# chaudatascience/diverse_channel_vit

Hardware: AMD Instinct MI355X
Metric: train images/sec, DiChaViT-S 8ch 224^2 bs=64/GPU (higher is better)
Workload: dtype bf16; 1 GPU; DiChaViT-small 8ch 224x224 P16 161 classes, train step (fwd + CE + ortho/proxy regularisers + bwd + fused AdamW), bs 64/GPU, N=1569 tokens; global_batch=64, seq_len=1569, parallelism=dp1, input=resident in HBM, launch=eager, wgrad_stream=False, wgrad_group=True

## Files before the change

### diverse_channel_vit_amd/csrc/gemm.hip

```cpp
#include <algorithm>
#include <atomic>
#include <type_traits>
#include "dcv_common.hpp"
#include "../../include/dcv.h"

namespace {

constexpr int BK = 64;

struct GemmNtArgs {
    const bf16_t* A;
    int lda;
    const bf16_t* W;
    int ldw;
    int M, N, K;
    const float* bias;
    void* out;
    int ldo;
    void* out2;
    int ldo2;
    const void* aux;
    int ldaux;
    const float* aux2;
    int T, n;
// ... 554 lines not shown
                const int c = 2 * hc + q;
                f32x4 va, vb;
#pragma unroll
                for (int r = 0; r < 4; ++r) {
                    float fa, fbv;
                    xchg_rows8(acc[i][2 * c][r], acc[i][2 * c + 1][r], fa, fbv);
                    va[r] = fa;
                    vb[r] = fbv;
                }
                const float bq[4] = {b4[q].x, b4[q].y, b4[q].z, b4[q].w};
                const float pa[4] = {xa[q].x, xa[q].y, xa[q].z, xa[q].w}, pb[4] = {xb[q].x, xb[q].y, xb[q].z, xb[q].w};
#pragma unroll
                for (int r = 0; r < 4; ++r) {
                    va[r] = fmaf(sa, va[r] + bq[r], pa[r]);
                    vb[r] = fmaf(sb, vb[r] + bq[r], pb[r]);
                }
                acc[i][2 * c] = va;
                acc[i][2 * c + 1] = vb;
                if (ma < a.M) *reinterpret_cast<f32x4*>((float*)a.out + (size_t)ma * a.ldo + ncol0 + 32 * c) = va;
                if (mb < a.M) *reinterpret_cast<f32x4*>((float*)a.out + (size_t)mb * a.ldo + ncol0 + 32 * c) = vb;
            }
        }
        float mu[2], m2[2];
#pragma unroll
        for (int h = 0; h < 2; ++h) {
            float s = 0.f;
#pragma unroll
            for (int c = 0; c < 6; ++c)
#pragma unroll
                for (int r = 0; r < 4; ++r) s += acc[i][2 * c + h][r];
            const float m = s * (1.f / 24.f);
            float q = 0.f;
#pragma unroll
            for (int c = 0; c < 6; ++c)
#pragma unroll
                for (int r = 0; r < 4; ++r) {
                    const float d = acc[i][2 * c + h][r] - m;
                    q = fmaf(d, d, q);
                }
            mu[h] = m;
            m2[h] = q;
        }
        float half_n = 12.f;
#pragma unroll
        for (int off = 8; off <= 32; off <<= 1) {
#pragma unroll
            for (int h = 0; h < 2; ++h) {
                const float om = __shfl_xor(mu[h], off, 64), oq = __shfl_xor(m2[h], off, 64);
                const float d = om - mu[h];
                m2[h] = m2[h] + oq + d * d * half_n;
                mu[h] = 0.5f * (mu[h] + om);
            }
            half_n *= 2.f;
        }
        if (hi == 0 && kg == 0) {
            const int rl = 16 * RB * wm + 16 * i + rr;
            *reinterpret_cast<float2*>(stat + ((size_t)(wn * 256 + rl) * 2)) = make_float2(mu[0], m2[0]);
            *reinterpret_cast<float2*>(stat + ((size_t)(wn * 256 + rl + 8) * 2)) = make_float2(mu[1], m2[1]);
        }
    }
    {
        const int t = 64 * (2 * wm + wn) + ln;
        if (t < 192) {
            const float4 v = *reinterpret_cast<const float4*>((t < 96 ? a.ln_g : a.ln_b) + 4 * (t < 96 ? t : t - 96));
            *reinterpret_cast<float4*>(stat + 1024 + 4 * t) = v;
        }
    }
    asm volatile("s_waitcnt lgkmcnt(0)" ::: "memory");
    __builtin_amdgcn_s_barrier();
    const int ln2 = lane_id_here();
    const int kg2 = ln2 >> 4, rr2 = ln2 & 7, hi2 = (ln2 >> 3) & 1;
    const int ncol2 = 192 * wn + 16 * hi2 + 4 * kg2;
#pragma unroll
    for (int i = 0; i < RB; ++i) {
        const int ma = m0 + 16 * RB * wm + 16 * i + rr2, mb = ma + 8;
        const int rl = 16 * RB * wm + 16 * i + rr2;
        float mean[2], rstd[2];
#pragma unroll
        for (int h = 0; h < 2; ++h) {
            const float2 p0 = *reinterpret_cast<const float2*>(stat + ((size_t)(rl + 8 * h) * 2));
            const float2 p1 = *reinterpret_cast<const float2*>(stat + ((size_t)(256 + rl + 8 * h) * 2));
            const float d = p1.x - p0.x;
            mean[h] = 0.5f * (p0.x + p1.x);
            rstd[h] = rsqrtf((p0.y + p1.y + d * d * 96.f) * (1.f / 384.f) + a.ln_eps);
        }
        if (wn == 0 && hi2 == 0 && kg2 == 0) {
            if (ma < a.M) { a.ln_mean[ma] = mean[0]; a.ln_rstd[ma] = rstd[0]; }
            if (mb < a.M) { a.ln_mean[mb] = mean[1]; a.ln_rstd[mb] = rstd[1]; }
        }
#pragma unroll
        for (int hc = 0; hc < 3; ++hc) {
            float4 g4[2], be4[2];
#pragma unroll
            for (int q = 0; q < 2; ++q) {
                g4[q] = *reinterpret_cast<const float4*>(stat + 1024 + ncol2 + 32 * (2 * hc + q));
                be4[q] = *reinterpret_cast<const float4*>(stat + 1024 + 384 + ncol2 + 32 * (2 * hc + q));
            }
            uint2 pa[2], pb[2];
#pragma unroll
            for (int q = 0; q < 2; ++q) {
                const int c = 2 * hc + q;
                const float g[4] = {g4[q].x, g4[q].y, g4[q].z, g4[q].w}, be[4] = {be4[q].x, be4[q].y, be4[q].z, be4[q].w};
                float ua[4], ub[4];
#pragma unroll
                for (int r = 0; r < 4; ++r) {
                    ua[r] = fmaf((acc[i][2 * c][r] - mean[0]) * rstd[0], g[r], be[r]);
                    ub[r] = fmaf((acc[i][2 * c + 1][r] - mean[1]) * rstd[1], g[r], be[r]);
                }
                pa[q] = pack4_bf16(ua[0], ua[1], ua[2], ua[3]);
                pb[q] = pack4_bf16(ub[0], ub[1], ub[2], ub[3]);
            }
            const u32x2_t ax = __builtin_amdgcn_permlane16_swap(pa[0].x, pa[1].x, false, false);
            const u32x2_t ay = __builtin_amdgcn_permlane16_swap(pa[0].y, pa[1].y, false, false);
            const u32x2_t bx = __builtin_amdgcn_permlane16_swap(pb[0].x, pb[1].x, false, false);
            const u32x2_t by = __builtin_amdgcn_permlane16_swap(pb[0].y, pb[1].y, false, false);
            const int kgp = kg2 & 1;
            const int ucol = 192 * wn + 32 * (2 * hc + kgp) + 16 * hi2 + 4 * (kg2 - kgp);
            if (ma < a.M) *reinterpret_cast<uint4*>((bf16_t*)a.out2 + (size_t)ma * a.ldo2 + ucol) = make_uint4(ax[0], ay[0], ax[1], ay[1]);
            if (mb < a.M) *reinterpret_cast<uint4*>((bf16_t*)a.out2 + (size_t)mb * a.ldo2 + ucol) = make_uint4(bx[0], by[0], bx[1], by[1]);
        }
    }
}

constexpr int N3_BM = 256, N3_BN = 384, N3_BK = 64;
constexpr int N3_A_BYTES = N3_BM * N3_BK * 2, N3_W_BYTES = N3_BN * N3_BK * 2, N3_STAGE_BYTES = N3_A_BYTES + N3_W_BYTES;
constexpr int N3_SMEM = 2 * N3_STAGE_BYTES;

template <int EPI>
__global__ __launch_bounds__(512) void gemm_nt384_kernel(GemmNtArgs a) {
    __shared__ __attribute__((aligned(16))) char smem[N3_SMEM];
    constexpr bool HAS_BIAS = (EPI != DCV_EPI_PLAIN_BF16) && (EPI != DCV_EPI_GELU_BWD_BF16);
    static_assert(EPI != DCV_EPI_PATCH, "the tokeniser epilogue stays on the 256 x 128 kernel");
    constexpr bool LN = (EPI == DCV_EPI_RESID_LN);
    constexpr int S1 = LN ? 0 : 3 * nt_stores_per_wave<LN ? DCV_EPI_BIAS_RESID_F32 : EPI>() / 4;
    const int tid = threadIdx.x, lane = tid & 63;
    const int wave = __builtin_amdgcn_readfirstlane(tid >> 6);
    const int wm = wave >> 1, wn = wave & 1;
    const bool late = (wave >> 2) != 0;
    const int tiles_n = a.N / N3_BN;
    const int total = a.tiles_m * tiles_n;
    const int G = gridDim.x;
    const int pos = ((G & 7) == 0) ? (blockIdx.x & 7) * (G >> 3) + (blockIdx.x >> 3) : blockIdx.x;

    const unsigned smem_base = __builtin_amdgcn_readfirstlane(lds_addr(smem));
    const unsigned dmaA = 32 * wave * 128, dmaW = N3_A_BYTES + 48 * wave * 128;
    const int nk = a.K / N3_BK;
    __builtin_assume(nk >= 1);
    const int r16 = lane & 15, kg = lane >> 4;
    const int rowA = (wm * 64 + r16) * 128, rowW = N3_A_BYTES + (wn * 192 + r16) * 128;
    int fA0, fA1, fW0, fW1;
    {
        const int co0 = (kg ^ swz64n(r16)) << 4;
        fA0 = rowA + co0; fA1 = rowA + (co0 ^ 64); fW0 = rowW + co0; fW1 = rowW + (co0 ^ 64);
        asm volatile("" : "+v"(fA0), "+v"(fA1), "+v"(fW0), "+v"(fW1));
    }

    unsigned voffA[2], voffW[2];
    auto set_voff = [&]() {
        const int ln = lane_id_here();
#pragma unroll
        for (int q = 0; q < 2; ++q) {
            const int rowa = 32 * wave + 8 * q + (ln >> 3), roww = 48 * wave + 8 * q + (ln >> 3);
            voffA[q] = (unsigned)(((size_t)rowa * a.lda + (((ln & 7) ^ swz64n(rowa)) * 8)) * 2);
            voffW[q] = (unsigned)(((size_t)roww * a.ldw + (((ln & 7) ^ swz64n(roww)) * 8)) * 2);
        }
    };
    set_voff();
    auto issue = [&](int m0_, int n0_, int h_, int kt, unsigned stage_base) {
        const int m0 = __builtin_amdgcn_readfirstlane(m0_), n0 = __builtin_amdgcn_readfirstlane(n0_);
        const int h = __builtin_amdgcn_readfirstlane(h_);
        const bf16_t* ab = a.A + (size_t)m0 * a.lda + kt * N3_BK;
        const bf16_t* wb = a.W + (size_t)n0 * a.ldw + kt * N3_BK;
        const bool has_rows = 32 * wave < h;
        if (has_rows && m0 + h <= a.M) {
#pragma unroll
            for (int q = 0; q < 4; ++q) glds16s(ab + (size_t)(q >> 1) * 16 * a.lda, voffA[q & 1], stage_base + dmaA + q * 1024);
        } else if (has_rows) {
            const int ln = lane_id_here();
#pragma unroll
            for (int q = 0; q < 4; ++q) {
                const int row = 32 * wave + 8 * q + (ln >> 3);
                const int rc = min(m0 + row, a.M - 1) - m0;
                glds16s(ab, (unsigned)(((size_t)rc * a.lda + (((ln & 7) ^ swz64n(row)) * 8)) * 2), stage_base + dmaA + q * 1024);
            }
        }
#pragma unroll
        for (int q = 0; q < 6; ++q) glds16s(wb + (size_t)(q >> 1) * 16 * a.ldw, voffW[q & 1], stage_base + dmaW + q * 1024);
    };

    auto tile_at = [&](int L_, int& m0_, int& n0_, int& h_) {
        const int tm = L_ / tiles_n, s192 = tm - a.n256;
        m0_ = s192 < 0 ? tm * N3_BM : a.n256 * N3_BM + s192 * 192;
        h_ = s192 < 0 ? N3_BM : 192;
        n0_ = (L_ - tm * tiles_n) * N3_BN;
    };
    int L = pos < total ? pos : -1;
    int Lnext = (L >= 0 && L + G < total) ? L + G : -1;
    if (L < 0) return;
    int m0, n0, h;
    tile_at(L, m0, n0, h);
    int g = 0;
    issue(m0, n0, h, 0, smem_base);
    int stores_behind = 0;

    auto tile = [&](auto rbc) __attribute__((always_inline)) -> bool {
        constexpr int RB = decltype(rbc)::value;
        constexpr int H = 64 * RB;
        f32x4 acc[RB][12];
#pragma unroll
        for (int i = 0; i < RB; ++i)
#pragma unroll
            for (int j = 0; j < 12; ++j)
#pragma unroll
                for (int r = 0; r < 4; ++r) acc[i][j][r] = 0.f;

#pragma clang loop unroll(disable)
        for (int kt = 0; kt < nk; ++kt, ++g) {
            if (kt == 0 && stores_behind == 4) asm volatile("s_waitcnt vmcnt(%0)" ::"n"(4 * S1) : "memory");
            else if (kt == 0 && stores_behind == 3) asm volatile("s_waitcnt vmcnt(%0)" ::"n"(3 * S1) : "memory");
            else asm volatile("s_waitcnt vmcnt(0)" ::: "memory");
            __builtin_amdgcn_s_barrier();
            const char* st = smem + (g & 1) * N3_STAGE_BYTES;
            const char* const stA = st - (4 - RB) * wm * 16 * 128;
            const char* const pA0 = stA + fA0;
            const char* const pA1 = stA + fA1;
            const char* const pW0 = st + fW0;
            const char* const pW1 = st + fW1;
            auto rdW = [&](int s2) { return as_bf16x8(lds_read128(s2 >= 12 ? pW1 : pW0, (s2 % 12) * 16 * 128)); };
            bf16x8 af[RB], wq[3];
#pragma unroll
            for (int i = 0; i < RB; ++i) af[i] = as_bf16x8(lds_read128(pA0, i * 16 * 128));
            wq[0] = rdW(0);
            wq[1] = rdW(1);
            __builtin_amdgcn_sched_barrier(0);
            if (kt + 1 < nk && (DCV_N3_EARLY_AT < 0 || late)) issue(m0, n0, H, kt + 1, smem_base + ((g + 1) & 1) * N3_STAGE_BYTES);
            __builtin_amdgcn_sched_barrier(0);
#pragma unroll
            for (int s2 = 0; s2 < 24; ++s2) {
                if (s2 + 2 < 24) wq[(s2 + 2) % 3] = rdW(s2 + 2);
#pragma unroll
                for (int i = 0; i < RB; ++i) {
                    acc[i][s2 % 12] = mfma16(wq[s2 % 3], af[i], acc[i][s2 % 12]);
                    if (s2 == 11) af[i] = as_bf16x8(lds_read128(pA1, i * 16 * 128));
                }
                __builtin_amdgcn_sched_barrier(0);
                if (DCV_N3_EARLY_AT >= 0 && s2 == DCV_N3_EARLY_AT) {
                    if (kt + 1 < nk && !late) issue(m0, n0, H, kt + 1, smem_base + ((g + 1) & 1) * N3_STAGE_BYTES);
                    __builtin_amdgcn_sched_barrier(0);
                }
            }
        }

        const int Ln = Lnext;
        const bool has_next = Ln >= 0;
        int m0n = 0, n0n = 0, hn = N3_BM;
        if (has_next) tile_at(Ln, m0n, n0n, hn);
        Lnext = (has_next && Ln + G < total) ? Ln + G : -1;
        const bool full = (m0 + H <= a.M);
        const int m_w = m0 + wm * 16 * RB, n_w = n0 + wn * 192;
        const int ln = lane_id_here();
        const int r16e = ln & 15, kge = ln >> 4;
        if constexpr (LN) {
            nt384_resid_ln_epilogue<RB>(a, acc, m0, wm, wn, ln, smem + ((g + 1) & 1) * N3_STAGE_BYTES, [&]() {
                if (has_next) issue(m0n, n0n, hn, 0, smem_base + (g & 1) * N3_STAGE_BYTES);
            });
        } else {
            auto block = [&](auto j0c, auto&& between) {
                constexpr int J0 = decltype(j0c)::value;
                float bz[8];
                if constexpr (HAS_BIAS) nt_load_bias<EPI, 4>(a, n_w + 16 * J0, r16e, kge, bz);
                nt_epilogue_block<EPI, 1, 4, 12, J0>(a, acc, m_w, n_w + 16 * J0, r16e, kge, bz, between);
            };
            block(std::integral_constant<int, 0>{}, [&]() {
                if (has_next) issue(m0n, n0n, hn, 0, smem_base + (g & 1) * N3_STAGE_BYTES);
            });
            block(std::integral_constant<int, 4>{}, []() {});
            block(std::integral_constant<int, 8>{}, []() {});
        }
        if (!has_next) return false;
        stores_behind = (full && !LN) ? RB : 0;
        m0 = m0n;
        n0 = n0n;
        h = hn;
        L = Ln;
        set_voff();
        return true;
    };
    for (;;) {
        if (h == N3_BM) {
            if (!tile(std::integral_constant<int, 4>{})) break;
        } else {
            if (!tile(std::integral_constant<int, 3>{})) break;
        }
    }
}

#ifndef DCV_NT_WS
#define DCV_NT_WS 1
#endif
#if DCV_NT_WS
constexpr int WS_BM = 32, WS_BN = 384, WS_K = 384, WS_WAVES = 12;
constexpr int WS_A_BYTES = WS_BM * WS_K * 2;
constexpr int WS_AUX_BYTES = WS_BM * WS_BN * 2;
template <int EPI>
struct WsCfg {
    static constexpr bool AUX = (EPI == DCV_EPI_GELU_BWD_BF16);
    static constexpr int STAGE = WS_A_BYTES + (AUX ? WS_AUX_BYTES : 0);
    static constexpr int NS = AUX ? 3 : 6;
    static constexpr int ND = AUX ? 4 : 2;
    static constexpr int S = 2 * (EPI == DCV_EPI_BIAS_GELU_BF16 ? 2 : 1);
    static constexpr int SMEM = NS * STAGE;
};

__device__ __forceinline__ void ws_wait_vm(int n) {
    switch (n) {
#define WS_W(k) \
    case k: asm volatile("s_waitcnt vmcnt(" #k ")" ::: "memory"); break;
        WS_W(0) WS_W(1) WS_W(2) WS_W(3) WS_W(4) WS_W(5) WS_W(6) WS_W(7) WS_W(8) WS_W(9) WS_W(10) WS_W(11) WS_W(12)
        WS_W(13) WS_W(14) WS_W(15) WS_W(16) WS_W(17) WS_W(18) WS_W(19) WS_W(20) WS_W(21) WS_W(22) WS_W(23) WS_W(24)
#undef WS_W
        default: asm volatile("s_waitcnt vmcnt(0)" ::: "memory"); break;
    }
}

template <int EPI>
__global__ __launch_bounds__(64 * WS_WAVES) void gemm_nt_ws_kernel(GemmNtArgs a) {
    using C = WsCfg<EPI>;
    __shared__ __attribute__((aligned(16))) char smem[C::SMEM];
    constexpr bool HAS_BIAS = (EPI == DCV_EPI_BIAS_BF16) || (EPI == DCV_EPI_BIAS_GELU_BF16);
    static_assert(EPI == DCV_EPI_BIAS_BF16 || EPI == DCV_EPI_BIAS_GELU_BF16 || EPI == DCV_EPI_PLAIN_BF16 || EPI == DCV_EPI_GELU_BWD_BF16,
                  "bf16-output epilogues only");
    const int tid = threadIdx.x, lane = tid & 63;
    const int wave = __builtin_amdgcn_readfirstlane(tid >> 6);
    const int r16 = lane & 15, kg = lane >> 4;
    const int slices = a.N / WS_BN;
    const int G = gridDim.x;
    const int groups = G / slices;
    const int q = xcd_remap(blockIdx.x, G);
    const int slice = q % slices, grp = q / slices;
    const int panels = (a.M + WS_BM - 1) / WS_BM;
    const int npl = grp < panels ? (panels - grp + groups - 1) / groups : 0;
    if (npl == 0) return;
    const int n0 = slice * WS_BN, nw = n0 + 32 * wave;
    const int ncol = nw + 16 * (kg & 1) + 8 * (kg >> 1);

    const unsigned smem_base = __builtin_amdgcn_readfirstlane(lds_addr(smem));
    int arow[2];
    unsigned acol[2], adst[2];
#pragma unroll
    for (int u = 0; u < 2; ++u) {
        const int p = 2 * wave + u, kc = p >> 2, row = 8 * (p & 3) + (lane >> 3);
        arow[u] = row;
        acol[u] = (unsigned)(64 * kc + (((lane & 7) ^ swz64n(row)) * 8)) * 2;
        adst[u] = kc * 4096 + (p & 3) * 1024;
    }
    auto issue = [&](int t) {
        const int m0 = __builtin_amdgcn_readfirstlane((grp + t * groups) * WS_BM);
        const unsigned slot = smem_base + (t % C::NS) * C::STAGE;
        const bf16_t* ab = a.A + (size_t)m0 * a.lda;
#pragma unroll
        for (int u = 0; u < 2; ++u) {
            const int rc = min(m0 + arow[u], a.M - 1) - m0;
            glds16s(ab, (unsigned)rc * a.lda * 2 + acol[u], slot + adst[u]);
        }
        if constexpr (C::AUX) {
            const bf16_t* xb = (const bf16_t*)a.aux + (size_t)m0 * a.ldaux;
#pragma unroll
            for (int i = 0; i < 2; ++i) {
                const int rc = min(m0 + 16 * i + r16, a.M - 1) - m0;
                glds16s(xb, (unsigned)(rc * a.ldaux + ncol) * 2, slot + WS_A_BYTES + (2 * wave + i) * 1024);
            }
        }
    };

    bf16x8 wf[2][12];
#pragma unroll
    for (int j = 0; j < 2; ++j) {
        const bf16_t* wr = a.W + (size_t)(nw + 16 * j + r16) * a.ldw + 8 * kg;
#pragma unroll
        for (int s = 0; s < 12; ++s) wf[j][s] = as_bf16x8(*reinterpret_cast<const uint4*>(wr + 32 * s));
    }
    float bz[8];
    if constexpr (HAS_BIAS) load8_f32(a.bias + ncol, bz);
#pragma unroll
    for (int t = 0; t < C::NS - 1; ++t)
        if (t < npl) issue(t);
#pragma unroll
    for (int j = 0; j < 2; ++j)
#pragma unroll
        for (int s = 0; s < 12; ++s) asm volatile("" : "+v"(wf[j][s]));
    if constexpr (HAS_BIAS) {
#pragma unroll
        for (int e = 0; e < 8; ++e) asm volatile("" : "+v"(bz[e]));
    }

    int fo0 = r16 * 128 + ((kg ^ swz64n(r16)) << 4);
    asm volatile("" : "+v"(fo0));
    const int fo1 = fo0 ^ 64;
    bool prev_full = false;
    for (int t = 0; t < npl; ++t) {
        const int ahead = min(C::NS - 2, npl - 1 - t);
        ws_wait_vm(C::ND * ahead + (prev_full ? C::S : 0));
        __builtin_amdgcn_s_barrier();
        if (t + C::NS - 1 < npl) issue(t + C::NS - 1);
        const int m0 = (grp + t * groups) * WS_BM;
        const char* st = smem + (t % C::NS) * C::STAGE;
        const char* const p0 = st + fo0;
        const char* const p1 = st + fo1;

        f32x4 acc[2][2];
#pragma unroll
        for (int i = 0; i < 2; ++i)
#pragma unroll
            for (int j = 0; j < 2; ++j)
#pragma unroll
                for (int r = 0; r < 4; ++r) acc[i][j][r] = 0.f;
        auto rdA = [&](int s, int i) { return as_bf16x8(lds_read128((s & 1) ? p1 : p0, (s >> 1) * 4096 + i * 2048)); };
        bf16x8 af[2][2];
        af[0][0] = rdA(0, 0);
        af[0][1] = rdA(0, 1);
#pragma unroll
        for (int s = 0; s < 12; ++s) {
            if (s + 1 < 12) {
                af[(s + 1) & 1][0] = rdA(s + 1, 0);
                af[(s + 1) & 1][1] = rdA(s + 1, 1);
            }
            __builtin_amdgcn_sched_barrier(0);
#pragma unroll
            for (int i = 0; i < 2; ++i)
#pragma unroll
                for (int j = 0; j < 2; ++j) acc[i][j] = mfma16(wf[j][s], af[s & 1][i], acc[i][j]);
            __builtin_amdgcn_sched_barrier(0);
        }

        const bool full = m0 + WS_BM <= a.M;
#pragma unroll
        for (int i = 0; i < 2; ++i) {
            float v[8], x[8];
            swap_pair8(acc[i][0], acc[i][1], v);
            if constexpr (C::AUX) unpack8_bf16(lds_read128(st + WS_A_BYTES, (2 * wave + i) * 1024 + lane * 16), x);
            const int m = m0 + 16 * i + r16;
            if (full || m < a.M) epi_store8<EPI>(a, m, ncol, v, x, bz);
        }
        prev_full = full;
    }
}
#endif

struct GemmTnArgs {
    const bf16_t* Y;
    int ldy;
    const bf16_t* X;
    int ldx;
    int M, P, Q;
    float* dW;
    int lddw;
    float* dbias;
    int m_per_split, splits;
    float* part;
    long part_stride;
    long bias_off;
};

__global__ __launch_bounds__(256) void gemm_tn_kernel(GemmTnArgs a) {
    __shared__ __attribute__((aligned(16))) char smem[2][2][BK * 128 * 2];
    const int tid = threadIdx.x, lane = tid & 63, wave = tid >> 6;
    const int wm = wave >> 1, wn = wave & 1;
    const int h = lane >> 5, r32 = lane & 31, li = lane & 15, g1 = (lane >> 4) & 1;
    const int tiles_q = (a.Q + 127) / 128;
    const int tiles = tiles_q * ((a.P + 127) / 128);
    int bid = xcd_remap(blockIdx.x, tiles * a.splits);
    const int split = bid / tiles;
    bid -= split * tiles;
    const int tq = bid % tiles_q, tp = bid / tiles_q;
    const int p0 = tp * 128, q0 = tq * 128;
    const int m_begin = split * a.m_per_split;
    const int m_end = min(a.M, m_begin + a.m_per_split);
    if (m_begin >= m_end) return;
    const int nk = (m_end - m_begin + BK - 1) / BK;

    const int srow = tid >> 4, sch = tid & 15;
    const int colY = min(p0 + sch * 8, a.P - 8), colX = min(q0 + sch * 8, a.Q - 8);
    int soff[4];
#pragma unroll
    for (int i = 0; i < 4; ++i) soff[i] = lds128_off(srow + 16 * i, sch * 8);
    const bf16_t* gY = a.Y + (size_t)colY;
    const bf16_t* gX = a.X + (size_t)colX;

    uint4 ry[4], rx[4];
    float bs0 = 0.f, bs1 = 0.f, bs2 = 0.f, bs3 = 0.f, bs4 = 0.f, bs5 = 0.f, bs6 = 0.f, bs7 = 0.f;
    const bool do_bias = (a.dbias != nullptr) && (tq == 0);

#define TN_LOAD_TILE(kt_)                                                                                          \
    _Pragma("unroll") for (int i = 0; i < 4; ++i) {                                                                \
        int m = m_begin + (kt_) * BK + srow + 16 * i;                                                              \
        const bool ok = m < m_end;                                                                                 \
        int mc = ok ? m : (m_end - 1);          \
        uint4 ty = *reinterpret_cast<const uint4*>(gY + (size_t)mc * a.ldy);                                       \
        uint4 tx = *reinterpret_cast<const uint4*>(gX + (size_t)mc * a.ldx);                                       \
        ry[i] = make_uint4(ok ? ty.x : 0u, ok ? ty.y : 0u, ok ? ty.z : 0u, ok ? ty.w : 0u);                        \
        rx[i] = make_uint4(ok ? tx.x : 0u, ok ? tx.y : 0u, ok ? tx.z : 0u, ok ? tx.w : 0u);                        \
    }
#define TN_STORE_TILE(buf_)                                                                                        \
    _Pragma("unroll") for (int i = 0; i < 4; ++i) {                                                                \
        lds_write128(smem[buf_][0], soff[i], ry[i]);                                                               \
        lds_write128(smem[buf_][1], soff[i], rx[i]);                                                               \
        if (do_bias) {                                                                                             \
            bs0 += __uint_as_float(ry[i].x << 16); bs1 += __uint_as_float(ry[i].x & 0xffff0000u);                  \
            bs2 += __uint_as_float(ry[i].y << 16); bs3 += __uint_as_float(ry[i].y & 0xffff0000u);                  \
            bs4 += __uint_as_float(ry[i].z << 16); bs5 += __uint_as_float(ry[i].z & 0xffff0000u);                  \
            bs6 += __uint_as_float(ry[i].w << 16); bs7 += __uint_as_float(ry[i].w & 0xffff0000u);                  \
        }                                                                                                          \
    }

    TN_LOAD_TILE(0)
    TN_STORE_TILE(0)
    __syncthreads();

    f32x16 acc[2][2];
#pragma unroll
    for (int i = 0; i < 2; ++i)
#pragma unroll
        for (int j = 0; j < 2; ++j)
#pragma unroll
            for (int r = 0; r < 16; ++r) acc[i][j][r] = 0.f;

    const int trow = 8 * h + (li >> 2);
    const int tcolA = wm * 64 + 16 * g1 + 4 * (li & 3);
    const int tcolB = wn * 64 + 16 * g1 + 4 * (li & 3);

    for (int kt = 0; kt < nk; ++kt) {
        const int cur = kt & 1;
        if (kt + 1 < nk) { TN_LOAD_TILE(kt + 1) }
        const char* sY = smem[cur][0];
        const char* sX = smem[cur][1];
#pragma unroll
        for (int ks = 0; ks < 4; ++ks) {
            const int row0 = 16 * ks + trow;
            bf16x8 af[2], bf[2];
#pragma unroll
            for (int i = 0; i < 2; ++i) {
                af[i] = join4(lds_tr_read(sY, lds128_off(row0, tcolA + 32 * i)), lds_tr_read(sY, lds128_off(row0 + 4, tcolA + 32 * i)));
                bf[i] = join4(lds_tr_read(sX, lds128_off(row0, tcolB + 32 * i)), lds_tr_read(sX, lds128_off(row0 + 4, tcolB + 32 * i)));
            }
#pragma unroll
            for (int i = 0; i < 2; ++i)
#pragma unroll
                for (int j = 0; j < 2; ++j) acc[i][j] = mfma32(af[i], bf[j], acc[i][j]);
        }
        if (kt + 1 < nk) { TN_STORE_TILE(cur ^ 1) }
        __syncthreads();
    }

#pragma unroll
    for (int i = 0; i < 2; ++i)
#pragma unroll
        for (int j = 0; j < 2; ++j) {
            const int q = q0 + wn * 64 + j * 32 + r32;
            if (q >= a.Q) continue;
#pragma unroll
            for (int r = 0; r < 16; ++r) {
                const int p = p0 + wm * 64 + i * 32 + acc_row(r, h);
                if (p < a.P) {
                    if (a.part) a.part[(size_t)split * a.part_stride + (size_t)p * a.Q + q] = acc[i][j][r];
                    else atomicAdd(a.dW + (size_t)p * a.lddw + q, acc[i][j][r]);
                }
            }
        }

    if (do_bias) {
        float* red = reinterpret_cast<float*>(smem[0][0]);
        float* rp = red + (srow * 16 + sch) * 8;
        rp[0] = bs0; rp[1] = bs1; rp[2] = bs2; rp[3] = bs3; rp[4] = bs4; rp[5] = bs5; rp[6] = bs6; rp[7] = bs7;
        __syncthreads();
        if (tid < 128) {
            int ch = tid >> 3, e = tid & 7;
            float s = 0.f;
#pragma unroll
            for (int rr = 0; rr < 16; ++rr) s += red[(rr * 16 + ch) * 8 + e];
            int p = p0 + ch * 8 + e;
            if (p < a.P) {
                if (a.part) a.part[(size_t)split * a.part_stride + (size_t)a.P * a.Q + p] = s;
                else atomicAdd(a.dbias + p, s);
            }
        }
    }
}

#ifndef DCV_T3_STAGES
#define DCV_T3_STAGES 4
#endif
constexpr int T3_BK = 32, T3_STAGES = DCV_T3_STAGES, T3_IMG = T3_BK * 256, T3_STAGE_BYTES = 4 * T3_IMG;

__device__ __forceinline__ void tn384_body(const GemmTnArgs& a, int bid, char* smem) {
    const int tid = threadIdx.x, lane = tid & 63;
    const int wave = __builtin_amdgcn_readfirstlane(tid >> 6);
    const int wp = wave >> 1, wq = wave & 1;
    const int h = lane >> 5, r32 = lane & 31, li = lane & 15, g1 = (lane >> 4) & 1;
    const int tiles_q = a.Q / 128, tiles = tiles_q * (a.P / 384);
    const int split = bid / tiles;
    bid -= split * tiles;
    const int tq = bid % tiles_q, tp = bid / tiles_q;
    const int p0 = tp * 384, q0 = tq * 128;
    const int m_begin = split * a.m_per_split;
    const int m_end = min(a.M, m_begin + a.m_per_split);
    if (m_begin >= m_end) return;
    const int nk = (m_end - m_begin + T3_BK - 1) / T3_BK;
    const int last_valid = (m_end - m_begin) - (nk - 1) * T3_BK;

    const int img = wave >> 1;
    const bf16_t* gsrc = (img < 3) ? a.Y + p0 + 128 * img : a.X + q0;
    const int ld = (img < 3) ? a.ldy : a.ldx;
    const int prow0 = 16 * (wave & 1) + (lane >> 4);
    int lc8[4];
#pragma unroll
    for (int j = 0; j < 4; ++j) {
        const int row = prow0 + 4 * j, pc = lane & 15;
        lc8[j] = (((((pc >> 2) ^ (row & 3)) << 2) | (pc & 3))) * 8;
    }
    const unsigned smem_base = __builtin_amdgcn_readfirstlane(lds_addr(smem));
    const unsigned dma_off = img * T3_IMG + 16 * (wave & 1) * 256;

#define T3_ISSUE(kt_)                                                                                     \
    {                                                                                                     \
        const unsigned sb_ = smem_base + ((kt_) % T3_STAGES) * T3_STAGE_BYTES + dma_off;                  \
        _Pragma("unroll") for (int j = 0; j < 4; ++j) {                                                   \
            const int m_ = min(m_begin + (kt_) * T3_BK + prow0 + 4 * j, m_end - 1);  \
            glds16(gsrc + (size_t)m_ * ld + lc8[j], sb_ + j * 1024);                                      \
        }                                                                                                 \
    }

    for (int st = 0; st < T3_STAGES - 1; ++st)
        if (st < nk) T3_ISSUE(st)

    f32x16 acc[3][2];
#pragma unroll
    for (int i = 0; i < 3; ++i)
#pragma unroll
        for (int j = 0; j < 2; ++j)
#pragma unroll
            for (int r = 0; r < 16; ++r) acc[i][j][r] = 0.f;

    const int trow = 8 * h + (li >> 2);
    int offA[3], offB[2];
#pragma unroll
    for (int i = 0; i < 3; ++i) {
        const int c = 96 * wp + 32 * i + 16 * g1 + 4 * (li & 3);
        offA[i] = (c >> 7) * T3_IMG + (c & 127);
    }
#pragma unroll
    for (int j = 0; j < 2; ++j) offB[j] = 3 * T3_IMG + (64 * wq + 32 * j + 16 * g1 + 4 * (li & 3));
    auto tr_off = [](int imgcol, int row) {
        const int base = imgcol & ~127, col = imgcol & 127;
        return base + lds128_off(row, col);
    };

    const bool do_bias = (a.dbias != nullptr);
    const int bch = tid % 48, brg = tid / 48;
    float bs[8];
#pragma unroll
    for (int e = 0; e < 8; ++e) bs[e] = 0.f;

    for (int kt = 0; kt < nk; ++kt) {
        const int rem = nk - 1 - kt;
        if (T3_STAGES >= 5 && rem >= 3) asm volatile("s_waitcnt vmcnt(12)" ::: "memory");
        else if (T3_STAGES >= 4 && rem >= 2) asm volatile("s_waitcnt vmcnt(8)" ::: "memory");
        else if (T3_STAGES >= 3 && rem >= 1) asm volatile("s_waitcnt vmcnt(4)" ::: "memory");
        else asm volatile("s_waitcnt vmcnt(0)" ::: "memory");
        __builtin_amdgcn_s_barrier();
        if (kt + T3_STAGES - 1 < nk) T3_ISSUE(kt + T3_STAGES - 1)
        char* st = smem + (kt % T3_STAGES) * T3_STAGE_BYTES;
        if (kt == nk - 1 && last_valid < T3_BK) {
            const int nbad = T3_BK - last_valid;
            for (int idx = tid; idx < nbad * 64; idx += 512) {
                const int r = last_valid + idx / 64, im = (idx & 63) >> 4, ch = idx & 15;
                lds_write128(st, im * T3_IMG + r * 256 + ch * 16, make_uint4(0, 0, 0, 0));
            }
            __syncthreads();
        }
#pragma unroll
        for (int ks = 0; ks < 2; ++ks) {
            const int row0 = 16 * ks + trow;
            bf16x8 af[3], bf[2];
#pragma unroll
            for (int i = 0; i < 3; ++i) af[i] = join4(lds_tr_read(st, tr_off(offA[i], row0)), lds_tr_read(st, tr_off(offA[i], row0 + 4)));
#pragma unroll
            for (int j = 0; j < 2; ++j) bf[j] = join4(lds_tr_read(st, tr_off(offB[j], row0)), lds_tr_read(st, tr_off(offB[j], row0 + 4)));
#pragma unroll
            for (int i = 0; i < 3; ++i)
#pragma unroll
                for (int j = 0; j < 2; ++j) acc[i][j] = mfma32(af[i], bf[j], acc[i][j]);
        }
        if (do_bias && (kt % tiles_q) == tq && brg < 10) {
            const int im = bch >> 4, ci = bch & 15;
            for (int r = brg; r < T3_BK; r += 10) {
                const int pc = ((((ci >> 2) ^ (r & 3)) << 2) | (ci & 3));
                const uint4 v = lds_read128(st, im * T3_IMG + r * 256 + pc * 16);
                bs[0] += __uint_as_float(v.x << 16); bs[1] += __uint_as_float(v.x & 0xffff0000u);
                bs[2] += __uint_as_float(v.y << 16); bs[3] += __uint_as_float(v.y & 0xffff0000u);
                bs[4] += __uint_as_float(v.z << 16); bs[5] += __uint_as_float(v.z & 0xffff0000u);
                bs[6] += __uint_as_float(v.w << 16); bs[7] += __uint_as_float(v.w & 0xffff0000u);
            }
        }
    }
#undef T3_ISSUE
#pragma unroll
    for (int i = 0; i < 3; ++i)
#pragma unroll
        for (int j = 0; j < 2; ++j) {
            const int q = q0 + wq * 64 + j * 32 + r32;
#pragma unroll
            for (int r = 0; r < 16; ++r) {
                const int p = p0 + wp * 96 + i * 32 + acc_row(r, h);
                if (a.part) a.part[(size_t)split * a.part_stride + (size_t)p * a.Q + q] = acc[i][j][r];
                else atomicAdd(a.dW + (size_t)p * a.lddw + q, acc[i][j][r]);
            }
        }
    if (do_bias) {
        __syncthreads();
        float* red = reinterpret_cast<float*>(smem);
        if (brg < 10) {
#pragma unroll
            for (int e = 0; e < 8; ++e) red[(brg * 48 + bch) * 8 + e] = bs[e];
        }
        __syncthreads();
        if (tid < 384) {
            float sum = 0.f;
#pragma unroll
            for (int g = 0; g < 10; ++g) sum += red[g * 384 + tid];
            if (a.part) a.part[a.bias_off + ((size_t)split * tiles_q + tq) * a.P + p0 + tid] = sum;
            else atomicAdd(a.dbias + p0 + tid, sum);
        }
    }
}

__global__ __launch_bounds__(512) void gemm_tn384_kernel(GemmTnArgs a) {
    __shared__ __attribute__((aligned(16))) char smem[T3_STAGES * T3_STAGE_BYTES];
    tn384_body(a, xcd_remap(blockIdx.x, (a.Q / 128) * (a.P / 384) * a.splits), smem);
}

constexpr int TN_GROUP_MAX = 8;
struct GemmTnGroup {
    int n;
    int start[TN_GROUP_MAX + 1];
    GemmTnArgs d[TN_GROUP_MAX];
// ... 394 lines not shown
```

Measured before the change: 1965 images/sec.

## Exchange epilogue tiles through LDS so waves write full 128-byte row lines

In the weight-stationary NT GEMM, the epilogue now packs results to bf16, exchanges half-tiles between paired waves via a small extra LDS area and DPP row swaps, and stores contiguous 64-column lines per row instead of scattered 16-byte pieces. By default it applies only to the GELU-backward epilogue, and stores use a streaming-store helper. The aim is better write coalescing into global memory. The cost is an extra LDS round trip and a workgroup barrier per tile, plus more LDS use. Ablation macros are added as well.

```diff
diff --git a/diverse_channel_vit_amd/csrc/gemm.hip b/diverse_channel_vit_amd/csrc/gemm.hip
--- a/diverse_channel_vit_amd/csrc/gemm.hip
+++ b/diverse_channel_vit_amd/csrc/gemm.hip
@@ -880,15 +880,76 @@
 constexpr int WS_BM = 32, WS_BN = 384, WS_K = 384, WS_WAVES = 12;
 constexpr int WS_A_BYTES = WS_BM * WS_K * 2;
 constexpr int WS_AUX_BYTES = WS_BM * WS_BN * 2;
+constexpr int WS_XA_BYTES = WS_WAVES * 1024;
+#ifndef DCV_WS_LINES
+#define DCV_WS_LINES 1
+#endif
+#ifndef DCV_WS_LINES_MASK
+#define DCV_WS_LINES_MASK (1 << DCV_EPI_GELU_BWD_BF16)
+#endif
+#ifndef DCV_WS_GELU_AREAS
+#define DCV_WS_GELU_AREAS 1
+#endif
+#ifndef DCV_WS_STREAM
+#define DCV_WS_STREAM 1
+#endif
+#ifndef DCV_WS_ABL
+#define DCV_WS_ABL 0
+#endif
 template <int EPI>
 struct WsCfg {
     static constexpr bool AUX = (EPI == DCV_EPI_GELU_BWD_BF16);
+    static constexpr bool LINES = DCV_WS_LINES && ((DCV_WS_LINES_MASK >> EPI) & 1);
+    static constexpr int XA = LINES ? ((EPI == DCV_EPI_BIAS_GELU_BF16 && DCV_WS_GELU_AREAS == 2) ? 2 : 1) : 0;
     static constexpr int STAGE = WS_A_BYTES + (AUX ? WS_AUX_BYTES : 0);
-    static constexpr int NS = AUX ? 3 : 6;
+    static constexpr int NS = AUX ? 3 : (XA == 2 ? 5 : 6);
     static constexpr int ND = AUX ? 4 : 2;
-    static constexpr int S = 2 * (EPI == DCV_EPI_BIAS_GELU_BF16 ? 2 : 1);
-    static constexpr int SMEM = NS * STAGE;
+    static constexpr int S = (DCV_WS_ABL & 1) ? 0 : 2 * (EPI == DCV_EPI_BIAS_GELU_BF16 ? 2 : 1);
+    static constexpr int RING = NS * STAGE;
+    static constexpr int SMEM = RING + XA * WS_XA_BYTES;
+    static_assert(SMEM <= 160 * 1024, "LDS");
 };
+__device__ __forceinline__ void ws_store128(void* p, uint4 v) {
+#if DCV_WS_ABL & 1
+    asm volatile("" ::"v"(p), "v"(v.x), "v"(v.y), "v"(v.z), "v"(v.w));
+#elif DCV_WS_STREAM
+    st128_stream(p, v);
+#else
+    *reinterpret_cast<uint4*>(p) = v;
+#endif
+}
+__device__ __forceinline__ void xchg_rows8_u4(const uint4& x, const uint4& y, uint4& a, uint4& b) {
+    a.x = __builtin_amdgcn_update_dpp(x.x, y.x, 0x128, 0xF, 0xC, false); b.x = __builtin_amdgcn_update_dpp(y.x, x.x, 0x128, 0xF, 0x3, false);
+    a.y = __builtin_amdgcn_update_dpp(x.y, y.y, 0x128, 0xF, 0xC, false); b.y = __builtin_amdgcn_update_dpp(y.y, x.y, 0x128, 0xF, 0x3, false);
+    a.z = __builtin_amdgcn_update_dpp(x.z, y.z, 0x128, 0xF, 0xC, false); b.z = __builtin_amdgcn_update_dpp(y.z, x.z, 0x128, 0xF, 0x3, false);
+    a.w = __builtin_amdgcn_update_dpp(x.w, y.w, 0x128, 0xF, 0xC, false); b.w = __builtin_amdgcn_update_dpp(y.w, x.w, 0x128, 0xF, 0x3, false);
+}
+template <int EPI>
+__device__ __forceinline__ void ws_epi_pack8(float* v, const float* x, const float* bz, uint4& pk, uint4& pk2) {
+    if constexpr (EPI == DCV_EPI_BIAS_BF16) {
+#pragma unroll
+        for (int e = 0; e < 8; ++e) v[e] += bz[e];
+        pk = pack8_bf16(v);
+    } else if constexpr (EPI == DCV_EPI_BIAS_GELU_BF16) {
+        float gp[8];
+#pragma unroll
+        for (int e = 0; e < 8; e += 2) {
+            const f32x2_t z = {v[e] + bz[e], v[e + 1] + bz[e + 1]};
+            f32x2_t g2, gp2;
+            gelu_parts2(z, g2, gp2);
+            v[e] = g2.x; v[e + 1] = g2.y;
+            gp[e] = gp2.x; gp[e + 1] = gp2.y;
+        }
+        pk = pack8_bf16(gp);
+        pk2 = pack8_bf16(v);
+    } else if constexpr (EPI == DCV_EPI_PLAIN_BF16) {
+        pk = pack8_bf16(v);
+    } else {
+#pragma unroll
+        for (int e = 0; e < 8; ++e) v[e] *= x[e];
+        pk = pack8_bf16(v);
+    }
+}
 
 __device__ __forceinline__ void ws_wait_vm(int n) {
     switch (n) {
@@ -921,6 +982,8 @@
     if (npl == 0) return;
     const int n0 = slice * WS_BN, nw = n0 + 32 * wave;
     const int ncol = nw + 16 * (kg & 1) + 8 * (kg >> 1);
+    const int odd = wave & 1, rr = r16 & 7;
+    const int nline = n0 + 64 * (wave >> 1) + 32 * (r16 >> 3) + 16 * (kg & 1) + 8 * (kg >> 1);
 
     const unsigned smem_base = __builtin_amdgcn_readfirstlane(lds_addr(smem));
     int arow[2];
@@ -977,10 +1040,10 @@
     const int fo1 = fo0 ^ 64;
     bool prev_full = false;
     for (int t = 0; t < npl; ++t) {
-        const int ahead = min(C::NS - 2, npl - 1 - t);
+        const int ahead = (DCV_WS_ABL & 2) ? 0 : min(C::NS - 2, npl - 1 - t);
         ws_wait_vm(C::ND * ahead + (prev_full ? C::S : 0));
         __builtin_amdgcn_s_barrier();
-        if (t + C::NS - 1 < npl) issue(t + C::NS - 1);
+        if (!(DCV_WS_ABL & 2) && t + C::NS - 1 < npl) issue(t + C::NS - 1);
         const int m0 = (grp + t * groups) * WS_BM;
         const char* st = smem + (t % C::NS) * C::STAGE;
         const char* const p0 = st + fo0;
@@ -1012,13 +1075,64 @@
         }
 
         const bool full = m0 + WS_BM <= a.M;
-#pragma unroll
-        for (int i = 0; i < 2; ++i) {
-            float v[8], x[8];
-            swap_pair8(acc[i][0], acc[i][1], v);
-            if constexpr (C::AUX) unpack8_bf16(lds_read128(st + WS_A_BYTES, (2 * wave + i) * 1024 + lane * 16), x);
-            const int m = m0 + 16 * i + r16;
-            if (full || m < a.M) epi_store8<EPI>(a, m, ncol, v, x, bz);
+        if constexpr (C::LINES) {
+            uint4 pk[2], pk2[2];
+#pragma unroll
+            for (int i = 0; i < 2; ++i) {
+                float v[8], x[8];
+                swap_pair8(acc[i][0], acc[i][1], v);
+                if constexpr (C::AUX) unpack8_bf16(lds_read128(st + WS_A_BYTES, (2 * wave + i) * 1024 + lane * 16), x);
+                ws_epi_pack8<EPI>(v, x, bz, pk[i], pk2[i]);
+            }
+            char* const xa = smem + C::RING;
+            const int mine = wave * 1024 + lane * 16, theirs = mine ^ 1024;
+            const int m = m0 + 16 * odd + rr;
+            const bool s0 = full || m < a.M, s1 = full || m + 8 < a.M;
+            lds_write128(xa, mine, odd ? pk[0] : pk[1]);
+            if constexpr (C::XA == 2) lds_write128(xa + WS_XA_BYTES, mine, odd ? pk2[0] : pk2[1]);
+            asm volatile("s_waitcnt lgkmcnt(0)" ::: "memory");
+            __builtin_amdgcn_s_barrier();
+            asm volatile("" ::: "memory");
+            auto store_lines = [&](void* o, int ld, const uint4& own, const uint4& got) {
+                uint4 va, vb;
+                xchg_rows8_u4(odd ? got : own, odd ? own : got, va, vb);
+                bf16_t* const ob = (bf16_t*)o + (size_t)m * ld + nline;
+                if (s0) ws_store128(ob, va);
+                if (s1) ws_store128(ob + (size_t)8 * ld, vb);
+            };
+            const uint4 got = lds_read128(xa, theirs);
+            if constexpr (EPI == DCV_EPI_BIAS_GELU_BF16 && C::XA == 2) {
+                const uint4 got2 = lds_read128(xa + WS_XA_BYTES, theirs);
+                store_lines(a.out, a.ldo, odd ? pk[1] : pk[0], got);
+                store_lines(a.out2, a.ldo2, odd ? pk2[1] : pk2[0], got2);
+            } else {
+                store_lines(a.out, a.ldo, odd ? pk[1] : pk[0], got);
+                if constexpr (EPI == DCV_EPI_BIAS_GELU_BF16) {
+                    lds_write128(xa, theirs, odd ? pk2[0] : pk2[1]);
+                    asm volatile("s_waitcnt lgkmcnt(0)" ::: "memory");
+                    __builtin_amdgcn_s_barrier();
+                    asm volatile("" ::: "memory");
+                    store_lines(a.out2, a.ldo2, odd ? pk2[1] : pk2[0], lds_read128(xa, mine));
+                }
+            }
+        } else {
+#pragma unroll
+            for (int i = 0; i < 2; ++i) {
+                float v[8], x[8];
+                swap_pair8(acc[i][0], acc[i][1], v);
+                if constexpr (C::AUX) unpack8_bf16(lds_read128(st + WS_A_BYTES, (2 * wave + i) * 1024 + lane * 16), x);
+                const int m = m0 + 16 * i + r16;
+#if !(DCV_WS_ABL & 1) && DCV_WS_STREAM
+                if (full || m < a.M) epi_store8<EPI>(a, m, ncol, v, x, bz);
+#else
+                if (full || m < a.M) {
+                    uint4 pk, pk2;
+                    ws_epi_pack8<EPI>(v, x, bz, pk, pk2);
+                    ws_store128((bf16_t*)a.out + (size_t)m * a.ldo + ncol, pk);
+                    if constexpr (EPI == DCV_EPI_BIAS_GELU_BF16) ws_store128((bf16_t*)a.out2 + (size_t)m * a.ldo2 + ncol, pk2);
+                }
+#endif
+            }
         }
         prev_full = full;
     }
```

Result: slower. 1945 images/sec (-1.0%).
